# vats98754/zero-knowledge-proofs

Measured on AMD Instinct MI355X. Metric: Groth16 prove constraints/sec at 2^20 R1CS; G1 MSM throughput (scalar-point/s), higher is better.
Workload: dtype u32; 1 GPU; groth16_prove_2^20; circuit=n x (x*y=z) (groth16-cli generate_crs), field=BLS12-381 Fq/Fr Montgomery, 32x32->64-bit limb products (radix 2^28/2^29), constraints=1048576, constraints_per_gpu=1048576, num_public=1, parallelism=single-gpu, quotient=local

## Files before the change

### zero-knowledge-proofs_amd/__init__.py

```python
import ctypes as C
import os

import numpy as np

_HERE = os.path.dirname(os.path.abspath(__file__))
LIB_PATH = os.environ.get("ZK_AMD_LIB") or os.path.join(_HERE, "libzkp_amd.so")
TEST_LIB_PATH = os.path.join(os.path.dirname(LIB_PATH), "libzkp_amd_test.so")

R = 0x73EDA753299D7D483339D80809A1D80553BDA402FFFE5BFEFFFFFFFF00000001

ZK_OK, ZK_ERR_MSM_LEN, ZK_ERR_INVALID_WITNESS, ZK_ERR_QAP_DIVISION, ZK_ERR_DOMAIN, \
    ZK_ERR_SETUP_PARAMS, ZK_ERR_DEVICE, ZK_ERR_RCCL, ZK_ERR_ARG, ZK_ERR_DIMENSION = range(10)
G1_WORDS, G2_WORDS = 13, 25
PARTIAL_BYTES = 1536

EXPORTS = (
    "zk_ctx_create", "zk_ctx_destroy", "zk_last_error", "zk_ctx_synchronize",
    "zk_ctx_profile", "zk_ctx_profile_read",
    "zk_msm_g1", "zk_msm_g2", "zk_msm_g1_upload", "zk_msm_g2_upload", "zk_msm_bases_free",
    "zk_msm_g1_dev", "zk_msm_g2_dev", "zk_ntt_fr", "zk_ntt_fr_dev",
    "zk_groth16_setup", "zk_groth16_setup_dev", "zk_pk_upload", "zk_pk_free",
    "zk_groth16_prove", "zk_groth16_prove_dev", "zk_pk_upload_shard",
    "zk_groth16_setup_dev_shard", "zk_groth16_prove_partial", "zk_groth16_prove_combine",
    "zk_proof_serialize_compressed", "zk_rccl_unique_id", "zk_ctx_attach_rccl",
# ... 8 lines not shown
    "zk_groth16_verify_many", "zk_pairing_products",
    "zk_groth16_setup_sound", "zk_groth16_setup_sound_dev", "zk_pk_upload_sound", "zk_pk_is_sound",
    "zk_groth16_verify_sound", "zk_groth16_verify_many_sound",
    "zk_msm_g1_upload_copies", "zk_msm_g2_upload_copies", "zk_pk_device_bytes",
    "zk_proofs_deserialize_compressed", "zk_groth16_verify_many_bytes", "zk_groth16_verify_many_bytes_sound",
    "zk_groth16_verify_all_sound", "zk_groth16_verify_all_bytes_sound",
    "zk_g1_mul_scalar", "zk_groth16_contribute_sound", "zk_groth16_verify_contribution_sound",
    "zk_srs_generate", "zk_g1_ntt", "zk_g2_ntt", "zk_groth16_setup_srs_sound", "zk_srs_verify",
    "zk_g1_mul_scalars", "zk_g2_mul_scalars", "zk_srs_contribute", "zk_srs_verify_contribution",
    "zk_sha256", "zk_hash_to_g2_host", "zk_hash_to_g2", "zk_pok_make", "zk_pok_verify", "zk_pok_verify_many",
    "zk_srs_digest", "zk_groth16_key_digest_sound", "zk_srs_prove_contribution",
    "zk_srs_verify_contribution_proofs",
    "zk_vk_prepare", "zk_vk_dev_free", "zk_vk_dev_bytes", "zk_vk_dev_is_sound", "zk_groth16_prepare_inputs",
    "zk_groth16_verify_many_prepared", "zk_groth16_verify_many_bytes_prepared",
)
TEST_EXPORTS = ("zk_test_prove_virtual_shards", "zk_test_exchange", "zk_test_fault_after_exchange",
                "zk_test_pk_bases", "zk_test_pk_info", "zk_test_pk_plan", "zk_test_fq_sqrt", "zk_test_fq2_sqrt",
                "zk_test_fq12", "zk_test_pairing_gt", "zk_test_fixed_base_g1", "zk_test_fixed_base_g2",
                "zk_test_verify_all_parts", "zk_test_g1_mul_scalar_plain",
                "zk_test_g1_mul_scalars_plain", "zk_test_g2_mul_scalars_plain", "zk_test_g1_mul_scalars_table",
                "zk_test_g2_mul_scalars_table", "zk_test_split_scalars", "zk_test_field", "zk_test_curve",
                "zk_test_gn_walk", "zk_test_hash_to_g2_capped", "zk_test_prepared_plan", "zk_test_prepared_run",
                "zk_test_prepared_force", "zk_test_prepared_info", "zk_test_msm_force", "zk_test_msm_info",
                "zk_test_msm_grouping", "zk_test_msm_scrub")
TEST_MSM_INFO = ("c", "nwin", "bits", "sw", "shared", "copies", "nred", "nseg", "segshift", "G", "T", "fix_max",
                 "M", "nbig", "natural_T", "n")
TEST_MSM_PART_G2, TEST_MSM_PART_ABI = 5, 6
ZK_OPT_QUOTIENT_PATH, ZK_OPT_PROVE_WIN_C, ZK_OPT_EXCHANGE_TIMEOUT_MS, ZK_OPT_DIST_QUOTIENT = 1, 2, 3, 5
ZK_OPT_EXCHANGE_FIRST = 6
ZK_OPT_POINT_CHUNK = 7
ZK_OPT_VERIFY_CHUNK = 8
ZK_OPT_SOUND_WIN_C = 9
ZK_OPT_SOUND_COPIES = 10
ZK_OPT_GNTT_MAP = 12
ZK_OPT_SRS_RUN = 13
ZK_VERIFY_REJECT, ZK_VERIFY_ACCEPT, ZK_VERIFY_MALFORMED = range(3)
(ZK_TEST_FQ12_MUL, ZK_TEST_FQ12_SQR, ZK_TEST_FQ12_INV, ZK_TEST_FQ12_CONJ, ZK_TEST_FQ12_FROB1, ZK_TEST_FQ12_FROB2,
 ZK_TEST_FQ12_CYC_SQR, ZK_TEST_FQ12_LINE_MUL, ZK_TEST_FQ12_FINAL_EXP) = range(9)
FINAL_EXP_C = 3
(ZK_TEST_FIELD_FR, ZK_TEST_FIELD_FQ, ZK_TEST_FIELD_FQ2, ZK_TEST_FIELD_FQ2H, ZK_TEST_FIELD_FQC,
 ZK_TEST_FIELD_FQ2C) = range(6)
(ZK_TEST_FOP_MUL, ZK_TEST_FOP_SQR, ZK_TEST_FOP_ADD, ZK_TEST_FOP_SUB, ZK_TEST_FOP_NEG, ZK_TEST_FOP_DBL,
 ZK_TEST_FOP_INV, ZK_TEST_FOP_TO_MONT, ZK_TEST_FOP_FROM_MONT, ZK_TEST_FOP_MUL_LAZY, ZK_TEST_FOP_MUL_SUB,
 ZK_TEST_FOP_FQ_INV, ZK_TEST_FOP_IS_ZERO) = range(13)
(ZK_TEST_COP_DBL, ZK_TEST_COP_DBL_CALL, ZK_TEST_COP_AFF_DBL, ZK_TEST_COP_MADD, ZK_TEST_COP_ADD,
 ZK_TEST_COP_ADD_ILP, ZK_TEST_COP_ADD_QUAD, ZK_TEST_COP_ADD_DUO) = range(8)
TEST_FIELD_WORDS = (8, 12, 24, 24, 12, 24)
# ... 565 lines not shown
    def prepare_inputs(self, pvk, inputs):
        if isinstance(inputs, np.ndarray) and inputs.ndim == 3:
            n = len(inputs)
        else:
            inputs = list(inputs)
            n = len(inputs)
        inp = self._verify_inputs(pvk, inputs, n)
        ic = np.zeros((n, G1_WORDS), dtype=np.uint64)
        ok = np.zeros(n, dtype=np.uint8)
        rc = lib().zk_groth16_prepare_inputs(C.c_void_p(self._h), pvk._handle(), _p(inp) if inp.size else None,
                                             C.c_size_t(inp.shape[1]), C.c_size_t(n), _p(ic) if n else None,
                                             _p(ok) if n else None)
        _check(rc, self, "zk_groth16_prepare_inputs")
        return ic, ok

    def test_prepared_force(self, width=0, run=0):
        _check(test_lib().zk_test_prepared_force(C.c_void_p(self._h), C.c_int(width), C.c_uint32(run)), self,
               "zk_test_prepared_force")

    def test_msm_force(self, T=0, fix_max=0):
        _check(test_lib().zk_test_msm_force(C.c_void_p(self._h), C.c_uint32(T), C.c_uint32(fix_max)), self,
               "zk_test_msm_force")

    def test_msm_scrub(self):
        _check(test_lib().zk_test_msm_scrub(C.c_void_p(self._h)), self, "zk_test_msm_scrub")

    def test_msm_info(self, which=0, g2=False):
        v = (C.c_uint32 * len(TEST_MSM_INFO))()
        _check(test_lib().zk_test_msm_info(C.c_void_p(self._h), C.c_int(which), C.c_int(1 if g2 else 0), v), self,
               "zk_test_msm_info")
        return dict(zip(TEST_MSM_INFO, (int(x) for x in v)))

    def test_msm_grouping(self, which=0):
        G, M = C.c_size_t(), C.c_size_t()
        fn = test_lib().zk_test_msm_grouping
        _check(fn(C.c_void_p(self._h), C.c_int(which), None, None, None, C.c_size_t(0), C.byref(G), C.byref(M)),
               self, "zk_test_msm_grouping")
        cap = max(G.value + 1, M.value)
        off, key, ent = (np.zeros(cap, dtype=np.uint32) for _ in range(3))
        _check(fn(C.c_void_p(self._h), C.c_int(which), _p(off), _p(key), _p(ent), C.c_size_t(cap), C.byref(G),
                  C.byref(M)), self, "zk_test_msm_grouping")
        return off[:G.value + 1], key[:M.value], ent[:M.value]

    @staticmethod
    def _proof_bytes(data, what):
        if isinstance(data, np.ndarray):
# ... 1507 lines not shown
```

### zero-knowledge-proofs_amd/csrc/group.hip

```cpp
#include "msm.hpp"

namespace zk {

#ifndef ZK_GS_THREADS
#define ZK_GS_THREADS 512
#endif
#ifndef ZK_GS_IPT
#define ZK_GS_IPT 16
#endif
constexpr uint32_t GS_THREADS = ZK_GS_THREADS;
constexpr uint32_t GS_WAVES = GS_THREADS / 64;
constexpr uint32_t GS_IPT = ZK_GS_IPT;
constexpr uint32_t GS_TE = GS_THREADS * GS_IPT;
constexpr uint32_t GS_WR = GS_IPT;
#ifndef ZK_GS_RB
#define ZK_GS_RB 8
#endif
constexpr uint32_t GS_MAXRB = ZK_GS_RB;
constexpr uint32_t GS_MAXNB = 1u << GS_MAXRB;
constexpr uint32_t GS_SCAN_ITEMS = 8;
constexpr uint32_t GS_SCAN_THREADS = 1024;
constexpr uint32_t GS_SCAN_CHUNK = GS_SCAN_ITEMS * GS_SCAN_THREADS;

struct GsArgs {
  const uint64_t* sc[MSM_MAXSEG];
  uint32_t n[MSM_MAXSEG], wstride[MSM_MAXSEG], ioff[MSM_MAXSEG], kbase[MSM_MAXSEG];
  uint32_t tile0[MSM_MAXSEG + 1];
  uint32_t boff[MSM_MAXWIN];
  uint32_t nseg, nwin, c, bits, shared, G, M, rb;
  uint32_t copies, setstride;
};

struct GsWin {
  uint32_t copy, ebase, kbase;
};
ZK_DI GsWin gs_next_win(const GsArgs& a, GsWin gw, uint32_t ioff, uint32_t wstride) {
  const bool wrap = gw.copy + 1 == a.copies;
  return {wrap ? 0u : gw.copy + 1, wrap ? ioff : gw.ebase + wstride, wrap ? gw.kbase + a.setstride : gw.kbase};
}

template <int SW>
ZK_DI uint32_t gs_digit(const GsArgs& a, uint32_t w, const uint64_t (&s)[SW], uint32_t& carry, bool& neg) {
  const bool top = w == a.nwin - 1;
  const int width = top ? (int)(a.bits - a.c * w) : (int)a.c;
  const uint32_t v = scal_window<SW>(s, (int)(a.c * w), width) + carry;
  if (!top && v > (1u << (a.c - 1))) {
    carry = 1;
    neg = true;
    return (1u << a.c) - v;
  }
  carry = 0;
  neg = false;
  return v;
}

ZK_DI void gs_entry(const GsArgs& a, GsWin gw, uint32_t i, uint32_t w, uint32_t mag, bool neg, uint32_t& key,
                    uint32_t& ent) {
  if (a.shared) {
    key = gw.kbase + (mag ? mag - 1 : 0u);
    ent = mag ? ((gw.ebase + i) | (neg ? 0x80000000u : 0u)) : MSM_DUMMY;
  } else {
    key = mag ? a.boff[w] + mag - 1 : a.G;
    ent = i | (neg ? 0x80000000u : 0u);
  }
}

ZK_DI uint32_t gs_seg(const GsArgs& a, uint32_t tile) {
  uint32_t k = 0;
#pragma unroll
  for (uint32_t j = 1; j < MSM_MAXSEG; j++)
    if (j < a.nseg && tile >= a.tile0[j]) k = j;
  return k;
}

template <int SW, bool SRC>
ZK_DI void gs_load(const GsArgs& a, uint32_t tile, const uint32_t* __restrict__ kin, const uint32_t* __restrict__ ein,
                   uint32_t (&key)[GS_IPT], uint32_t (&ent)[GS_IPT], uint32_t& valid) {
  const uint32_t lane = threadIdx.x & 63, wave = threadIdx.x >> 6;
  valid = 0;
  if constexpr (SRC) {
    const uint32_t k = gs_seg(a, tile);
    const uint32_t u0 = (tile - a.tile0[k]) * (GS_TE / 64) + wave * GS_WR;
    const uint32_t nk = a.n[k];
    uint32_t pr = u0 / a.nwin, w = u0 - pr * a.nwin;
    uint32_t i = pr * 64 + lane;
    uint64_t s[SW];
    uint32_t carry = 0;
    bool neg = false;
#pragma unroll
    for (int j = 0; j < SW; j++) s[j] = i < nk ? a.sc[k][(size_t)i * SW + j] : 0ull;
    const uint32_t ioff = a.ioff[k], wstride = a.wstride[k];
    const GsWin gw0{0u, ioff, a.kbase[k]};
    GsWin gw = gw0;
    for (uint32_t q = 0; q < w; q++) {
      (void)gs_digit<SW>(a, q, s, carry, neg);
      gw = gs_next_win(a, gw, ioff, wstride);
    }
#pragma unroll
    for (uint32_t r = 0; r < GS_IPT; r++) {
      key[r] = ent[r] = 0;
      if (i < nk) {
        const uint32_t mag = gs_digit<SW>(a, w, s, carry, neg);
        gs_entry(a, gw, i, w, mag, neg, key[r], ent[r]);
        valid |= 1u << r;
      }
      gw = gs_next_win(a, gw, ioff, wstride);
      if (++w == a.nwin) {
        w = 0;
        carry = 0;
        gw = gw0;
        i += 64;
#pragma unroll
        for (int j = 0; j < SW; j++) s[j] = (r + 1 < GS_IPT && i < nk) ? a.sc[k][(size_t)i * SW + j] : 0ull;
      }
    }
  } else {
    const size_t e0 = (size_t)tile * GS_TE + wave * GS_WR * 64 + lane;
#pragma unroll
    for (uint32_t r = 0; r < GS_IPT; r++) {
      const size_t e = e0 + 64 * r;
      const bool ok = e < a.M;
      key[r] = ok ? kin[e] : 0u;
      ent[r] = ok ? ein[e] : 0u;
      if (ok) valid |= 1u << r;
    }
  }
}

template <int SW, bool SRC>
__global__ void __launch_bounds__(GS_THREADS) k_gs_count(GsArgs a, uint32_t shift, uint32_t ntiles,
                                                         const uint32_t* __restrict__ kin,
                                                         uint32_t* __restrict__ cnt) {
  __shared__ uint32_t h[GS_MAXNB];
  const uint32_t NB = 1u << a.rb, tile = blockIdx.x;
  for (uint32_t b = threadIdx.x; b < NB; b += GS_THREADS) h[b] = 0;
  __syncthreads();
  uint32_t key[GS_IPT], ent[GS_IPT], valid;
  if constexpr (SRC) {
    gs_load<SW, true>(a, tile, nullptr, nullptr, key, ent, valid);
  } else {
    const size_t e0 = (size_t)tile * GS_TE + (threadIdx.x >> 6) * GS_WR * 64 + (threadIdx.x & 63);
    valid = 0;
#pragma unroll
    for (uint32_t r = 0; r < GS_IPT; r++) {
// ... 143 lines not shown
    for (uint32_t bit = 0; bit < a.rb; bit++) {
      const uint64_t bb = __ballot((d >> bit) & 1u);
      m &= ((d >> bit) & 1u) ? bb : ~bb;
    }
    if (ok) {
      const uint32_t base = wh[wave][d];
      const uint32_t slot = base + __popcll(m & lt_mask);
      sk[slot] = key[r];
      se[slot] = ent[r];
      if ((m & lt_mask) == 0) wh[wave][d] = base + __popcll(m);
      cnt++;
    }
  }
  uint32_t tot = 0;
  (void)gs_block_scan<GS_THREADS>(cnt, ws, &tot);
  for (uint32_t j = threadIdx.x; j < tot; j += GS_THREADS) {
    const uint32_t k = sk[j];
    const uint32_t g = tb[(k >> shift) & (NB - 1)] + j;
    kout[g] = k;
    eout[g] = se[j];
  }
}

constexpr uint32_t OFF_LONG_RUN = 64;
__global__ void __launch_bounds__(256) k_msm_offsets(const uint32_t* __restrict__ key, uint32_t M, uint32_t G,
                                                     uint32_t* __restrict__ off, uint32_t* __restrict__ ctl) {
  __shared__ uint32_t run_lo[256], run_hi[256], run_i[256], nrun;
  const uint32_t i = blockIdx.x * blockDim.x + threadIdx.x;
  if (i < 2) ctl[i] = 0;
  if (threadIdx.x == 0) nrun = 0;
  __syncthreads();
  if (i <= M) {
    const uint32_t lo = i ? min(key[i - 1], G) + 1 : 0;
    const uint32_t hi = i < M ? min(key[i], G) : G;
    if (lo <= hi && hi - lo >= OFF_LONG_RUN) {
      const uint32_t r = atomicAdd(&nrun, 1u);
      run_lo[r] = lo;
      run_hi[r] = hi;
      run_i[r] = i;
    } else {
      for (uint32_t g = lo; g <= hi; g++) off[g] = i;
    }
  }
  __syncthreads();
  for (uint32_t r = 0; r < nrun; r++)
    for (uint32_t g = run_lo[r] + threadIdx.x; g <= run_hi[r]; g += 256) off[g] = run_i[r];
}

void msm_offsets(MsmWork& w, uint32_t M, hipStream_t st) {
  w.nbig.ensure(2 * sizeof(uint32_t));
  k_msm_offsets<<<ceil_div((uint64_t)M + 1, 256), 256, 0, st>>>(w.key.as<uint32_t>(), M, w.plan.G,
                                                                 w.off.as<uint32_t>(), w.nbig.as<uint32_t>());
  ZK_LAUNCH_CHECK();
}

template <int SW>
static void gs_run(MsmWork& w, const GsArgs& a, uint32_t ntiles0, hipStream_t st) {
  const MsmPlan& p = w.plan;
  const uint32_t M = a.M;
  uint32_t maxkey = p.shared ? p.G - 1 : p.G;
  uint32_t kb = 1;
  while (kb < 32 && (maxkey >> kb)) kb++;
  const uint32_t P = (kb + GS_MAXRB - 1) / GS_MAXRB;
  GsArgs g = a;
  g.rb = (kb + P - 1) / P;
  const uint32_t NB = 1u << g.rb;
  const uint32_t ntiles1 = ceil_div(M, GS_TE);
  const size_t L = (size_t)NB * std::max(ntiles0, ntiles1);
  w.gcnt.ensure(sizeof(uint32_t) * std::max<size_t>(L, 1));
  w.gcnt_sums.ensure(sizeof(uint32_t) * (L / GS_SCAN_CHUNK + 2));
  uint32_t* cnt = w.gcnt.as<uint32_t>();
  uint32_t* sums = w.gcnt_sums.as<uint32_t>();
  uint32_t* kbuf[2] = {w.key.as<uint32_t>(), w.key_in.as<uint32_t>()};
  uint32_t* ebuf[2] = {w.ent.as<uint32_t>(), w.ent_in.as<uint32_t>()};
  const uint32_t* kin = nullptr;
  const uint32_t* ein = nullptr;
  for (uint32_t pass = 0; pass < P; pass++) {
    const uint32_t shift = pass * g.rb;
    const uint32_t nt = pass == 0 ? ntiles0 : ntiles1;
    const size_t Lp = (size_t)NB * nt;
    if (pass == 0)
      k_gs_count<SW, true><<<nt, GS_THREADS, 0, st>>>(g, shift, nt, nullptr, cnt);
    else
      k_gs_count<SW, false><<<nt, GS_THREADS, 0, st>>>(g, shift, nt, kin, cnt);
    ZK_LAUNCH_CHECK();
    const uint32_t nchunk = ceil_div(Lp, GS_SCAN_CHUNK);
    k_gs_scan_sums<<<nchunk, GS_SCAN_THREADS, 0, st>>>(cnt, Lp, sums);
    ZK_LAUNCH_CHECK();
// ... 20 lines not shown
  a.shared = p.shared ? 1u : 0u;
  a.G = p.G;
  a.copies = p.shared ? (uint32_t)p.copies : 1u;
  a.setstride = p.nb[0];
  for (int k = 0; k < p.nwin && k < MSM_MAXWIN; k++) a.boff[k] = p.boff[k];
  uint32_t tiles = 0;
  size_t M = 0;
  for (int k = 0; k < nseg; k++) {
    a.sc[k] = segs[k].scalars;
    a.n[k] = segs[k].n;
    a.wstride[k] = segs[k].wstride ? segs[k].wstride : segs[k].n;
    a.ioff[k] = segs[k].ioff;
    a.kbase[k] = (p.shared && nseg > 1) ? (uint32_t)k << (p.segshift & 31) : 0u;
    a.tile0[k] = tiles;
    const uint64_t rounds = (uint64_t)ceil_div(segs[k].n, 64) * (uint64_t)p.nwin;
    tiles += (uint32_t)((rounds + GS_TE / 64 - 1) / (GS_TE / 64));
    M += (size_t)segs[k].n * p.nwin;
  }
  for (int k = nseg; k <= MSM_MAXSEG; k++) a.tile0[k] = tiles;
  a.M = (uint32_t)M;
  if (M) {
    w.key_in.ensure(sizeof(uint32_t) * M);
    w.ent_in.ensure(sizeof(uint32_t) * M);
    if (sw == 1) gs_run<1>(w, a, tiles, st);
    else gs_run<4>(w, a, tiles, st);
  }
  msm_offsets(w, (uint32_t)M, st);
}

}
```

### zero-knowledge-proofs_amd/csrc/msm.hip

```cpp
#include <algorithm>
#include <cstdlib>
#include <cstring>
#include <type_traits>
#include <vector>

#include "msm.hpp"

namespace zk {

MsmPlan msm_make_plan(uint32_t n, int bits, int sw, int force_c) {
  MsmPlan p{};
  p.n = n;
  p.bits = bits;
  p.sw = sw;
  int best_c = 4;
  double best = 1e300;
  for (int nw = (bits + 15) / 16; nw <= std::min(MSM_MAXWIN, bits); nw++) {
    const int c = (bits + nw - 1) / nw;
    if (c < 4) break;
    const int nwin = (bits + c - 1) / c;
    const int top = bits - c * (nwin - 1);
    const double nbuck = (double)(nwin - 1) * (1u << (c - 1)) + (double)(1u << top);
    const double cost = (double)n * nwin + 3.5 * nbuck;
    if (cost < best) { best = cost; best_c = c; }
// ... 668 lines not shown
  const uint32_t n = p.n;
  (void)n;
  int ph = pf ? pf->begin(st, (w.tag + "msm_merge").c_str(), p.G) : -1;
  const bool by_boundary = p.G > p.T;
  const size_t fix_n = by_boundary ? p.T : p.G;
  k_msm_fixup<C><<<ceil_div(Lanes<C>::N * fix_n, 128), 128, 0, st>>>(
      w.key.as<uint32_t>(), w.off.as<uint32_t>(), p.G, p.T, p.fix_max, by_boundary, w.nbig.as<uint32_t>(),
      w.buckets.as<X>(), w.partials.as<X>());
  ZK_LAUNCH_CHECK();
  {
    uint32_t nlevels = 0;
    while ((1ull << (ZK_MERGE_FAN_LOG * nlevels)) < p.T) nlevels++;
    const uint32_t groups1 = (uint32_t)(((uint64_t)p.T + MSM_MERGE_FAN - 1) >> ZK_MERGE_FAN_LOG);
    if (nlevels) {
      const uint32_t grid = std::min<uint32_t>(std::min<uint32_t>(ceil_div(groups1, 128), 64), merge_max_blocks<C>());
      if (grid < 1 || grid > merge_max_blocks<C>()) throw Error(ZK_ERR_DEVICE, "msm: merge grid exceeds residency");
      k_msm_merge<C><<<grid, 128, 0, st>>>(
          w.key.as<uint32_t>(), w.off.as<uint32_t>(), p.G, p.T, p.fix_max, nlevels, w.nbig.as<uint32_t>(),
          w.buckets.as<X>(), w.partials.as<X>(), w.partials2.as<X>());
      ZK_LAUNCH_CHECK();
    }
  }
  p.all_valid = 0;
  if (mode == MSM_BACK_COMBINE || mode == MSM_BACK_ACCUM) {
    if (!prev || prev->plan.G != p.G || prev->plan.nseg != p.nseg) throw Error(ZK_ERR_ARG, "msm: combine plans differ");
    const bool prev_all = prev->plan.all_valid != 0;
    k_msm_combine<C><<<ceil_div(Lanes<C>::N * (size_t)p.G, 128), 128, 0, st>>>(
        w.off.as<uint32_t>(), prev->off.as<uint32_t>(), prev_all, p.G, w.buckets.as<X>(), prev->buckets.as<X>());
    ZK_LAUNCH_CHECK();
    p.all_valid = 1;
  }
  if (pf) pf->end(st, ph);
  if (mode == MSM_BACK_FIXUP || mode == MSM_BACK_ACCUM) return;
  ph = pf ? pf->begin(st, (w.tag + "msm_bucket_sum").c_str(), p.G) : -1;
  k_msm_rowcol<C><<<ceil_div(p.nrc, MSM_RED_WAVES), 64 * MSM_RED_WAVES, 0, st>>>(p, w.off.as<uint32_t>(),
                                                                                w.buckets.as<X>(), w.rc.as<X>());
  ZK_LAUNCH_CHECK();
  constexpr int RW = g2 ? ZK_QUANT_WAVES_G2 : ZK_QUANT_WAVES_G1;
  k_msm_quant<C, RW><<<p.nq, 64 * RW, 0, st>>>(p, w.rc.as<X>(), w.res.as<X>());
  ZK_LAUNCH_CHECK();
  if (pf) pf->end(st, ph);
}

template <class C>
void msm_launch(MsmWork& w, const typename C::A* d_bases, const uint64_t* d_scalars, int sw, uint32_t n,
                int bits, hipStream_t st, uint32_t stride) {
  w.plan = msm_make_plan(n, bits, sw);
  const MsmSeg seg{d_bases, d_scalars, n, stride};
// ... 120 lines not shown
  out[t] = k < iw ? in[i * iw + k] : make_uint4(0, 0, 0, 0);
}

template <class C>
uint32_t msm_pad_bases(DevBuf& d, size_t n, hipStream_t st) {
  constexpr uint32_t sz = sizeof(typename C::A), padded = (sz + 127) / 128 * 128;
  if (padded == sz) return 0;
  DevBuf out;
  out.ensure((size_t)padded * std::max<size_t>(n, 1));
  if (n) {
    k_pad_copy<<<ceil_div(n * (padded / 16), 256), 256, 0, st>>>(d.as<uint4>(), n, sz / 16, padded / 16,
                                                                  out.as<uint4>());
    ZK_LAUNCH_CHECK();
  }
  ZK_HIP(hipStreamSynchronize(st));
  d = std::move(out);
  return padded;
}

template <class C>
void msm_download(MsmWork& w, hipStream_t st) {
  using X = typename C::X;
  const size_t bytes = sizeof(X) * w.plan.nq;
  w.host_res.ensure(bytes);
  ZK_HIP(hipMemcpyAsync(w.host_res.p, w.res.p, bytes, hipMemcpyDeviceToHost, st));
}

template <class C>
static host::X<typename C::HF> msm_finish_impl(const MsmWork& w, int seg) {
  using HF = typename C::HF;
  using HX = host::X<HF>;
  static_assert(sizeof(HX) == sizeof(typename C::X), "layout");
  const MsmPlan& p = w.plan;
  const HX* r = w.host_res.as<const HX>();
  auto wexp = [&](int win) { return !p.shared ? p.c * win : p.nseg > 1 ? 0 : p.c * p.copies * win; };
  const int w0 = seg < 0 ? 0 : seg, w1 = seg < 0 ? (int)p.nred : seg + 1;
  int maxe = 0;
  for (int win = w0; win < w1; win++)
    maxe = std::max(maxe, wexp(win) + std::max<int>(p.kc[win] + p.kr[win] - 1, p.kc[win]));
  std::vector<std::vector<const HX*>> at(maxe + 1);
  for (int win = w0; win < w1; win++) {
    const int kr = p.kr[win], kc = p.kc[win];
    for (int q = 0; q < kr + kc + 1; q++) {
      int e = q < kr ? wexp(win) + kc + q : q < kr + kc ? wexp(win) + (q - kr) : wexp(win);
      at[e].push_back(&r[p.qoff[win] + q]);
    }
  }
  HX acc = host::inf<HF>();
  auto host_form = [](const HX& d) {
    return HX{host::to_host(d.X_), host::to_host(d.Y), host::to_host(d.ZZ), host::to_host(d.ZZZ)};
  };
  for (int e = maxe; e >= 0; e--) {
    acc = host::dbl(acc);
    for (const HX* t : at[e]) acc = host::addp(acc, host_form(*t));
  }
  return acc;
}
// ... 104 lines not shown
```

### zero-knowledge-proofs_amd/csrc/msm.hpp

```cpp
#pragma once
#include <string>
#include <vector>

#include "common.hpp"
#include "curve.hpp"
#include "host_ec.hpp"

namespace zk {

template <int SW>
__device__ __forceinline__ uint32_t scal_window(const uint64_t (&s)[SW], int off, int width) {
  int wd = off >> 6, sh = off & 63;
  uint64_t lo = 0;
#pragma unroll
  for (int k = 0; k < SW; k++)
    if (k == wd) lo = s[k] >> sh;
  if (sh + width > 64) {
#pragma unroll
    for (int k = 0; k < SW; k++)
      if (k == wd + 1) lo |= s[k] << (64 - sh);
  }
  return (uint32_t)(lo & ((1ull << width) - 1));
}

// ... 38 lines not shown

constexpr int MSM_MAXSEG = 4;
struct MsmSeg {
  const void* bases;
  const uint64_t* scalars;
  uint32_t n;
  uint32_t stride = 0;
  uint32_t wstride = 0, ioff = 0;
};

MsmPlan msm_make_plan(uint32_t n, int bits, int sw, int force_c = 0);
struct MsmWork;
struct MsmSeg;
void msm_group(MsmWork& w, const MsmSeg* segs, int nseg, int sw, hipStream_t st);
void msm_offsets(MsmWork& w, uint32_t M, hipStream_t st);
MsmPlan msm_make_plan_shared(uint32_t n, int bits, int sw, int c);
MsmPlan msm_make_plan_grouped(uint32_t n, int bits, int sw, int c, int copies);

struct MsmWork {
  DevBuf off, ent, key, buckets, partials, partials2, rc, res;
  DevBuf key_in, ent_in;
  DevBuf nbig;
  DevBuf gcnt, gcnt_sums;
  PinnedBuf host_res;
  MsmPlan plan{};
  Prof* prof = nullptr;
  std::string tag;
  uint32_t force_T = 0, force_fix_max = 0;
};

template <class C>
uint32_t msm_accum_units();

template <class C>
void msm_launch(MsmWork& w, const typename C::A* d_bases, const uint64_t* d_scalars, int sw,
                uint32_t n, int bits, hipStream_t st, uint32_t stride = 0);
template <class C>
void msm_launch_grouped(MsmWork& w, const typename C::A* d_bases, const uint64_t* d_scalars, int sw,
                        uint32_t n, int bits, int c, int copies, hipStream_t st, uint32_t stride = 0);
template <class C>
void msm_launch_batch(MsmWork& w, const MsmSeg* segs, int nseg, int bits, int c, hipStream_t st);
enum { MSM_BACK_FULL = 0, MSM_BACK_FIXUP = 1, MSM_BACK_COMBINE = 2, MSM_BACK_ACCUM = 3 };
template <class C>
void msm_batch_front(MsmWork& w, const MsmSeg* segs, int nseg, int bits, int c, hipStream_t st);
template <class C>
void msm_batch_back(MsmWork& w, hipStream_t st, int mode, const MsmWork* prev);
template <class C>
void msm_precompute_windows(typename C::A* d_bases, size_t n, int W, int c, hipStream_t st);
template <class C>
uint32_t msm_pad_bases(DevBuf& d, size_t n, hipStream_t st);
template <class C>
void batch_normalize(const typename C::X* d_in, size_t n, typename C::F* d_pre, typename C::A* d_out,
// ... 19 lines not shown
```

### zero-knowledge-proofs_amd/csrc/testhooks.hip

```cpp
#include <algorithm>
#include <cstring>
#include <vector>

#include "ceremony.hpp"
#include "ctx.hpp"
#include "hash.hpp"
#include "msm.hpp"
#include "mulvec.hpp"
#include "pairing.hpp"
#include "points.hpp"
#include "prepared.hpp"
#include "prove.hpp"
#include "setup.hpp"
#include "verify_all.hpp"
#include "../../include/zkp_test.h"

using namespace zk;

#define ZK_TGUARD(ctx, ...)                                   \
  try {                                                       \
    ZK_HIP(hipSetDevice((ctx)->device));                      \
    __VA_ARGS__                                               \
  } catch (const zk::Error& e) {                              \
    (ctx)->err = e.what();                                    \
// ... 793 lines not shown
  return nullptr;
}
static void test_msm_sync(zk_ctx* ctx) {
  ZK_HIP(hipStreamSynchronize(ctx->stream));
  for (int k = 0; k < NUM_SIDE; k++)
    if (ctx->side[k]) ZK_HIP(hipStreamSynchronize(ctx->side[k]));
}
static bool test_msm_ran(const MsmWork& w) { return w.plan.G && w.off.p && w.nbig.p && w.key.p && w.ent.p; }
}

int zk_test_msm_force(zk_ctx* ctx, uint32_t T, uint32_t fix_max) {
  if (!ctx || T > (1u << 22)) return ZK_ERR_ARG;
  for (int k = 0; k < NUM_MSM; k++) {
    ctx->msm[k].force_T = T;
    ctx->msm[k].force_fix_max = fix_max;
  }
  for (int k = 0; k < HOST_PARTS - 1; k++) {
    ctx->part_g2[k].force_T = ctx->part_abi[k].force_T = T;
    ctx->part_g2[k].force_fix_max = ctx->part_abi[k].force_fix_max = fix_max;
  }
  return ZK_OK;
}

int zk_test_msm_info(zk_ctx* ctx, int which, int g2, uint32_t* info) {
  if (!ctx || !info || (g2 != 0 && g2 != 1)) return ZK_ERR_ARG;
  MsmWork* w = test_msm_work(ctx, which);
  if (!w) return ZK_ERR_ARG;
  ZK_TGUARD(ctx, {
    if (!test_msm_ran(*w)) throw Error(ZK_ERR_ARG, "test_msm_info: no MSM has run on this workspace");
    const MsmPlan& p = w->plan;
    test_msm_sync(ctx);
    uint32_t M = 0, nbig = 0;
    ZK_HIP(hipMemcpy(&M, w->off.as<uint32_t>() + p.G, sizeof(uint32_t), hipMemcpyDeviceToHost));
    ZK_HIP(hipMemcpy(&nbig, w->nbig.p, sizeof(uint32_t), hipMemcpyDeviceToHost));
    info[ZK_TEST_MSM_C] = (uint32_t)p.c;
    info[ZK_TEST_MSM_NWIN] = (uint32_t)p.nwin;
    info[ZK_TEST_MSM_BITS] = (uint32_t)p.bits;
    info[ZK_TEST_MSM_SW] = (uint32_t)p.sw;
    info[ZK_TEST_MSM_SHARED] = (uint32_t)p.shared;
    info[ZK_TEST_MSM_COPIES] = (uint32_t)p.copies;
    info[ZK_TEST_MSM_NRED] = p.nred;
    info[ZK_TEST_MSM_NSEG] = (uint32_t)p.nseg;
    info[ZK_TEST_MSM_SEGSHIFT] = p.segshift;
    info[ZK_TEST_MSM_G] = p.G;
    info[ZK_TEST_MSM_T] = p.T;
    info[ZK_TEST_MSM_FIX_MAX] = p.fix_max;
// ... 49 lines not shown
```

Before: 123.7 million constraints/s.

## Fuse MSM bucket radix sort with decoupled lookback and segmented key passes

Replaces the multi-kernel radix grouping of MSM bucket keys with a fused scheme. One histogram kernel computes the digit counts for every pass and the global base offsets at once. Each pass kernel then scatters using a single-pass decoupled lookback over per-tile status words, with ticket-ordered tiles. For batched shared-window MSMs it also sorts per segment on fewer key bits, which can reduce the number of passes. The cost is spin-waiting between workgroups, guarded by a poll limit and an error flag checked on the host, plus extra control memory.

```diff
diff --git a/zero-knowledge-proofs_amd/__init__.py b/zero-knowledge-proofs_amd/__init__.py
--- a/zero-knowledge-proofs_amd/__init__.py
+++ b/zero-knowledge-proofs_amd/__init__.py
@@ -54,7 +54,8 @@
                 "zk_test_g2_mul_scalars_table", "zk_test_split_scalars", "zk_test_field", "zk_test_curve",
                 "zk_test_gn_walk", "zk_test_hash_to_g2_capped", "zk_test_prepared_plan", "zk_test_prepared_run",
                 "zk_test_prepared_force", "zk_test_prepared_info", "zk_test_msm_force", "zk_test_msm_info",
-                "zk_test_msm_grouping", "zk_test_msm_scrub")
+                "zk_test_msm_grouping", "zk_test_msm_scrub", "zk_test_group_force",
+                "zk_test_msm_batch_front", "zk_test_group_info")
 TEST_MSM_INFO = ("c", "nwin", "bits", "sw", "shared", "copies", "nred", "nseg", "segshift", "G", "T", "fix_max",
                  "M", "nbig", "natural_T", "n")
 TEST_MSM_PART_G2, TEST_MSM_PART_ABI = 5, 6
@@ -666,6 +667,23 @@
         _check(test_lib().zk_test_msm_force(C.c_void_p(self._h), C.c_uint32(T), C.c_uint32(fix_max)), self,
                "zk_test_msm_force")
 
+    def test_group_force(self, mode=0):
+        _check(test_lib().zk_test_group_force(C.c_void_p(self._h), C.c_int(mode)), self, "zk_test_group_force")
+
+    def test_group_info(self, which=0):
+        f, e = C.c_uint32(), C.c_uint32()
+        _check(test_lib().zk_test_group_info(C.c_void_p(self._h), C.c_int(which), C.byref(f), C.byref(e)), self,
+               "zk_test_group_info")
+        return bool(f.value), int(e.value)
+
+    def test_msm_batch_front(self, scalars, sizes):
+        sc = np.ascontiguousarray(scalars, dtype=np.uint64).reshape(-1)
+        n = np.asarray(sizes, dtype=np.uint32)
+        if int(n.sum()) != len(sc):
+            raise ValueError("test_msm_batch_front: sizes do not add up to the scalars")
+        _check(test_lib().zk_test_msm_batch_front(C.c_void_p(self._h), _p(sc) if len(sc) else None, _p(n),
+                                                  C.c_int(len(n))), self, "zk_test_msm_batch_front")
+
     def test_msm_scrub(self):
         _check(test_lib().zk_test_msm_scrub(C.c_void_p(self._h)), self, "zk_test_msm_scrub")
 
diff --git a/zero-knowledge-proofs_amd/csrc/group.hip b/zero-knowledge-proofs_amd/csrc/group.hip
--- a/zero-knowledge-proofs_amd/csrc/group.hip
+++ b/zero-knowledge-proofs_amd/csrc/group.hip
@@ -18,6 +18,9 @@
 #endif
 constexpr uint32_t GS_MAXRB = ZK_GS_RB;
 constexpr uint32_t GS_MAXNB = 1u << GS_MAXRB;
+#ifndef ZK_GS_SEGMENTED
+#define ZK_GS_SEGMENTED 1
+#endif
 constexpr uint32_t GS_SCAN_ITEMS = 8;
 constexpr uint32_t GS_SCAN_THREADS = 1024;
 constexpr uint32_t GS_SCAN_CHUNK = GS_SCAN_ITEMS * GS_SCAN_THREADS;
@@ -26,6 +29,7 @@
   const uint64_t* sc[MSM_MAXSEG];
   uint32_t n[MSM_MAXSEG], wstride[MSM_MAXSEG], ioff[MSM_MAXSEG], kbase[MSM_MAXSEG];
   uint32_t tile0[MSM_MAXSEG + 1];
+  uint32_t tile1[MSM_MAXSEG + 1], soff[MSM_MAXSEG + 1], nts;
   uint32_t boff[MSM_MAXWIN];
   uint32_t nseg, nwin, c, bits, shared, G, M, rb;
   uint32_t copies, setstride;
@@ -70,6 +74,13 @@
 #pragma unroll
   for (uint32_t j = 1; j < MSM_MAXSEG; j++)
     if (j < a.nseg && tile >= a.tile0[j]) k = j;
+  return k;
+}
+ZK_DI uint32_t gs_seg1(const GsArgs& a, uint32_t tile) {
+  uint32_t k = 0;
+#pragma unroll
+  for (uint32_t j = 1; j < MSM_MAXSEG; j++)
+    if (j < a.nts && tile >= a.tile1[j]) k = j;
   return k;
 }
 
@@ -115,11 +126,13 @@
       }
     }
   } else {
-    const size_t e0 = (size_t)tile * GS_TE + wave * GS_WR * 64 + lane;
+    const uint32_t k = gs_seg1(a, tile);
+    const size_t e0 = a.soff[k] + (size_t)(tile - a.tile1[k]) * GS_TE + wave * GS_WR * 64 + lane;
+    const size_t end = a.soff[k + 1];
 #pragma unroll
     for (uint32_t r = 0; r < GS_IPT; r++) {
       const size_t e = e0 + 64 * r;
-      const bool ok = e < a.M;
+      const bool ok = e < end;
       key[r] = ok ? kin[e] : 0u;
       ent[r] = ok ? ein[e] : 0u;
       if (ok) valid |= 1u << r;
@@ -309,11 +322,225 @@
   }
 }
 
+constexpr uint32_t GS_MAXP = 4;
+constexpr uint32_t GS_CTL_ERR = 0, GS_CTL_ARRIVED = 1, GS_CTL_TICKET = 2, GS_CTL_HIST = 8;
+constexpr uint32_t GS_HIST_WORDS = GS_MAXP * MSM_MAXSEG * GS_MAXNB;
+constexpr uint32_t GS_CTL_BASE = GS_CTL_HIST + GS_HIST_WORDS;
+constexpr uint32_t GS_CTL_STAT = GS_CTL_BASE + GS_HIST_WORDS;
+constexpr bool GS_FUSED_OK = GS_MAXNB <= GS_THREADS && GS_MAXRB * GS_MAXP >= 32;
+
+constexpr uint32_t GS_ST_SHIFT = 30, GS_ST_MASK = (1u << GS_ST_SHIFT) - 1;
+constexpr uint32_t GS_ST_AGG = 1, GS_ST_INCL = 2, GS_ST_BLOCK = 3;
+constexpr uint32_t GS_LB = 16;
+constexpr uint32_t GS_BLK = 32;
+constexpr uint32_t GS_POLL_MAX = 1u << 20;
+
+#ifndef ZK_GS_RELEASE
+#define ZK_GS_RELEASE 0
+#endif
+ZK_DI void gs_publish(uint32_t* p, uint32_t state, uint32_t count) {
+  __hip_atomic_store(p, state << GS_ST_SHIFT | count, ZK_GS_RELEASE ? __ATOMIC_RELEASE : __ATOMIC_RELAXED,
+                     __HIP_MEMORY_SCOPE_AGENT);
+}
+
+template <uint32_t STEP>
+ZK_DI bool gs_walk(uint32_t* stat, uint32_t NB, uint32_t b, uint32_t pos, uint32_t n, uint32_t& sum, bool& incl) {
+  uint32_t polls = 0;
+  while (n && !incl) {
+    uint32_t wv[GS_LB];
+#pragma unroll
+    for (uint32_t j = 0; j < GS_LB; j++)
+      wv[j] = j < n ? __hip_atomic_load(&stat[(size_t)(pos - STEP * j) * NB + b], __ATOMIC_RELAXED,
+                                        __HIP_MEMORY_SCOPE_AGENT)
+                    : 0u;
+    bool stall = false;
+    uint32_t adv = 0;
+#pragma unroll
+    for (uint32_t j = 0; j < GS_LB; j++) {
+      const uint32_t st = wv[j] >> GS_ST_SHIFT;
+      if (j < n && !incl && !stall) {
+        if (STEP == 1 ? st == 0 : st < GS_ST_INCL) {
+          stall = true;
+        } else {
+          sum += wv[j] & GS_ST_MASK;
+          adv++;
+          incl = st == GS_ST_INCL;
+        }
+      }
+    }
+    n -= adv;
+    pos -= STEP * adv;
+    if (stall) {
+      if (++polls > GS_POLL_MAX) return false;
+      __builtin_amdgcn_s_sleep(4);
+    }
+  }
+  return true;
+}
+
+ZK_DI bool gs_lookback(uint32_t* stat, uint32_t NB, uint32_t b, uint32_t first, uint32_t tile, uint32_t tc,
+                       uint32_t& excl) {
+  const uint32_t rel = tile - first, blk = rel / GS_BLK, in_blk = rel % GS_BLK;
+  uint32_t sum = 0;
+  bool incl = false;
+  if (!gs_walk<1>(stat, NB, b, tile - 1, in_blk, sum, incl)) return false;
+  if (!incl && blk) {
+    if (in_blk == GS_BLK - 1) gs_publish(&stat[(size_t)tile * NB + b], GS_ST_BLOCK, sum + tc);
+    if (!gs_walk<GS_BLK>(stat, NB, b, tile - in_blk - 1, blk, sum, incl)) return false;
+  }
+  if (ZK_GS_RELEASE) __builtin_amdgcn_fence(__ATOMIC_ACQUIRE, "agent");
+  excl = sum;
+  return true;
+}
+
+template <int SW>
+__global__ void __launch_bounds__(GS_THREADS) k_gs_hist(GsArgs a, uint32_t P, uint32_t nrows,
+                                                        uint32_t* __restrict__ ctl) {
+  __shared__ uint32_t h[GS_MAXP][GS_MAXNB];
+  __shared__ uint32_t ws[GS_THREADS / 64 + 1];
+  __shared__ uint32_t last;
+  const uint32_t NB = 1u << a.rb, tile = blockIdx.x;
+  for (uint32_t j = threadIdx.x; j < GS_MAXP * GS_MAXNB; j += GS_THREADS) (&h[0][0])[j] = 0;
+  __syncthreads();
+  uint32_t key[GS_IPT], ent[GS_IPT], valid;
+  gs_load<SW, true>(a, tile, nullptr, nullptr, key, ent, valid);
+  (void)ent;
+#pragma unroll
+  for (uint32_t r = 0; r < GS_IPT; r++)
+    if (valid >> r & 1u)
+      for (uint32_t p = 0; p < P; p++) atomicAdd(&h[p][(key[r] >> (p * a.rb)) & (NB - 1)], 1u);
+  __syncthreads();
+  uint32_t* hist = ctl + GS_CTL_HIST;
+  const uint32_t reg = a.nts > 1 ? gs_seg(a, tile) : 0u;
+  for (uint32_t j = threadIdx.x; j < P * NB; j += GS_THREADS) {
+    const uint32_t p = j >> a.rb, b = j & (NB - 1), c = h[p][b];
+    if (c) __hip_atomic_fetch_add(&hist[(p * MSM_MAXSEG + reg) * GS_MAXNB + b], c, __ATOMIC_RELAXED,
+                                  __HIP_MEMORY_SCOPE_AGENT);
+  }
+  uint32_t* stat = ctl + GS_CTL_STAT;
+  const size_t nstat = (size_t)2 * nrows * NB;
+  for (size_t j = (size_t)blockIdx.x * GS_THREADS + threadIdx.x; j < nstat; j += (size_t)gridDim.x * GS_THREADS)
+    stat[j] = 0;
+  __threadfence();
+  __syncthreads();
+  if (threadIdx.x == 0)
+    last = __hip_atomic_fetch_add(&ctl[GS_CTL_ARRIVED], 1u, __ATOMIC_ACQ_REL, __HIP_MEMORY_SCOPE_AGENT) ==
+           gridDim.x - 1;
+  __syncthreads();
+  if (!last) return;
+  __threadfence();
+  uint32_t* base = ctl + GS_CTL_BASE;
+  for (uint32_t p = 0; p < P; p++)
+    for (uint32_t k = 0; k < a.nts; k++) {
+      uint32_t* hp = &hist[(p * MSM_MAXSEG + k) * GS_MAXNB];
+      uint32_t c = 0;
+      if (threadIdx.x < NB) {
+        c = __hip_atomic_load(&hp[threadIdx.x], __ATOMIC_RELAXED, __HIP_MEMORY_SCOPE_AGENT);
+        __hip_atomic_store(&hp[threadIdx.x], 0u, __ATOMIC_RELAXED, __HIP_MEMORY_SCOPE_AGENT);
+      }
+      const uint32_t ex = gs_block_scan<GS_THREADS>(c, ws, nullptr);
+      if (threadIdx.x < NB) base[(p * MSM_MAXSEG + k) * GS_MAXNB + threadIdx.x] = a.soff[k] + ex;
+    }
+  if (threadIdx.x < GS_MAXP) ctl[GS_CTL_TICKET + threadIdx.x] = 0;
+  if (threadIdx.x == 0) ctl[GS_CTL_ERR] = ctl[GS_CTL_ARRIVED] = 0;
+}
+
+template <int SW, bool SRC>
+__global__ void __launch_bounds__(GS_THREADS) k_gs_pass(GsArgs a, uint32_t pass, uint32_t* __restrict__ ctl,
+                                                        uint32_t* __restrict__ stat, uint32_t* __restrict__ clr,
+                                                        const uint32_t* __restrict__ kin,
+                                                        const uint32_t* __restrict__ ein,
+                                                        uint32_t* __restrict__ kout, uint32_t* __restrict__ eout) {
+  static_assert(GS_MAXNB <= GS_THREADS || !GS_FUSED_OK, "a thread per bin");
+  __shared__ uint32_t sk[GS_TE], se[GS_TE];
+  __shared__ uint32_t wh[GS_WAVES][GS_MAXNB];
+  __shared__ uint32_t tb[GS_MAXNB];
+  __shared__ uint32_t ws[GS_THREADS / 64 + 1];
+  __shared__ uint32_t my_tile, gave_up;
+  const uint32_t NB = 1u << a.rb, shift = pass * a.rb;
+  const uint32_t lane = threadIdx.x & 63, wave = threadIdx.x >> 6;
+  if (threadIdx.x == 0) {
+    my_tile = __hip_atomic_fetch_add(&ctl[GS_CTL_TICKET + pass], 1u, __ATOMIC_RELAXED, __HIP_MEMORY_SCOPE_AGENT);
+    gave_up = 0;
+  }
+  for (uint32_t j = threadIdx.x; j < GS_WAVES * GS_MAXNB; j += GS_THREADS) (&wh[0][0])[j] = 0;
+  __syncthreads();
+  const uint32_t tile = my_tile;
+  uint32_t reg = 0, first = 0;
+  if (a.nts > 1) {
+    reg = SRC ? gs_seg(a, tile) : gs_seg1(a, tile);
+    first = SRC ? a.tile0[reg] : a.tile1[reg];
+  }
+  uint32_t key[GS_IPT], ent[GS_IPT], valid;
+  gs_load<SW, SRC>(a, tile, kin, ein, key, ent, valid);
+#pragma unroll
+  for (uint32_t r = 0; r < GS_IPT; r++)
+    if (valid >> r & 1u) atomicAdd(&wh[wave][(key[r] >> shift) & (NB - 1)], 1u);
+  __syncthreads();
+  const uint32_t b = threadIdx.x;
+  uint32_t tc = 0;
+  if (b < NB) {
+    for (uint32_t v = 0; v < GS_WAVES; v++) {
+      const uint32_t c = wh[v][b];
+      wh[v][b] = tc;
+      tc += c;
+    }
+    gs_publish(&stat[(size_t)tile * NB + b], tile == first ? GS_ST_INCL : GS_ST_AGG, tc);
+    if (clr) clr[(size_t)tile * NB + b] = 0;
+  }
+  const uint32_t lb = gs_block_scan<GS_THREADS>(tc, ws, nullptr);
+  if (b < NB) {
+    uint32_t excl = 0;
+    if (tile != first) {
+      if (gs_lookback(stat, NB, b, first, tile, tc, excl)) {
+        gs_publish(&stat[(size_t)tile * NB + b], GS_ST_INCL, excl + tc);
+      } else {
+        __hip_atomic_store(&ctl[GS_CTL_ERR], 1u, __ATOMIC_RELAXED, __HIP_MEMORY_SCOPE_AGENT);
+        gave_up = 1;
+      }
+    }
+    tb[b] = ctl[GS_CTL_BASE + (pass * MSM_MAXSEG + reg) * GS_MAXNB + b] + excl - lb;
+    for (uint32_t v = 0; v < GS_WAVES; v++) wh[v][b] += lb;
+  }
+  __syncthreads();
+  if (gave_up) return;
+  const uint64_t lt_mask = (1ull << lane) - 1;
+  uint32_t cnt = 0;
+#pragma unroll
+  for (uint32_t r = 0; r < GS_IPT; r++) {
+    const bool ok = valid >> r & 1u;
+    const uint32_t d = (key[r] >> shift) & (NB - 1);
+    uint64_t m = __ballot(ok);
+    for (uint32_t bit = 0; bit < a.rb; bit++) {
+      const uint64_t bb = __ballot((d >> bit) & 1u);
+      m &= ((d >> bit) & 1u) ? bb : ~bb;
+    }
+    if (ok) {
+      const uint32_t base = wh[wave][d];
+      const uint32_t slot = base + __popcll(m & lt_mask);
+      sk[slot] = key[r];
+      se[slot] = ent[r];
+      if ((m & lt_mask) == 0) wh[wave][d] = base + __popcll(m);
+      cnt++;
+    }
+  }
+  uint32_t tot = 0;
+  (void)gs_block_scan<GS_THREADS>(cnt, ws, &tot);
+  for (uint32_t j = threadIdx.x; j < tot; j += GS_THREADS) {
+    const uint32_t k = sk[j];
+    const uint32_t g = tb[(k >> shift) & (NB - 1)] + j;
+    kout[g] = k;
+    eout[g] = se[j];
+  }
+}
+
 constexpr uint32_t OFF_LONG_RUN = 64;
 __global__ void __launch_bounds__(256) k_msm_offsets(const uint32_t* __restrict__ key, uint32_t M, uint32_t G,
-                                                     uint32_t* __restrict__ off, uint32_t* __restrict__ ctl) {
+                                                     uint32_t* __restrict__ off, uint32_t* __restrict__ ctl,
+                                                     const uint32_t* __restrict__ err) {
   __shared__ uint32_t run_lo[256], run_hi[256], run_i[256], nrun;
   const uint32_t i = blockIdx.x * blockDim.x + threadIdx.x;
+  if (err && *err) M = 0;
   if (i < 2) ctl[i] = 0;
   if (threadIdx.x == 0) nrun = 0;
   __syncthreads();
@@ -336,9 +563,67 @@
 
 void msm_offsets(MsmWork& w, uint32_t M, hipStream_t st) {
   w.nbig.ensure(2 * sizeof(uint32_t));
+  const uint32_t* err = w.group_fused ? w.gctl.as<uint32_t>() + GS_CTL_ERR : nullptr;
   k_msm_offsets<<<ceil_div((uint64_t)M + 1, 256), 256, 0, st>>>(w.key.as<uint32_t>(), M, w.plan.G,
-                                                                 w.off.as<uint32_t>(), w.nbig.as<uint32_t>());
+                                                                 w.off.as<uint32_t>(), w.nbig.as<uint32_t>(), err);
   ZK_LAUNCH_CHECK();
+}
+
+template <int SW>
+static void gs_run_fused(MsmWork& w, const GsArgs& a, uint32_t ntiles0, hipStream_t st) {
+  const MsmPlan& p = w.plan;
+  GsArgs g = a;
+  const bool batch = a.nseg > 1 && a.shared && ZK_GS_SEGMENTED;
+  uint32_t kb = 1;
+  if (batch) {
+    kb = p.segshift;
+  } else {
+    const uint32_t maxkey = p.shared ? p.G - 1 : p.G;
+    while (kb < 32 && (maxkey >> kb)) kb++;
+  }
+  const uint32_t P = (kb + GS_MAXRB - 1) / GS_MAXRB;
+  g.rb = (kb + P - 1) / P;
+  const uint32_t NB = 1u << g.rb;
+  g.nts = batch ? a.nseg : 1u;
+  uint32_t ntiles1 = 0, at = 0;
+  for (uint32_t k = 0; k < g.nts; k++) {
+    const uint32_t len = batch ? a.n[k] * a.nwin : a.M;
+    g.soff[k] = at;
+    g.tile1[k] = ntiles1;
+    at += len;
+    ntiles1 += ceil_div(len, GS_TE);
+  }
+  for (uint32_t k = g.nts; k <= MSM_MAXSEG; k++) {
+    g.soff[k] = at;
+    g.tile1[k] = ntiles1;
+  }
+  const uint32_t nrows = std::max(ntiles0, ntiles1);
+  const size_t words = GS_CTL_STAT + (size_t)2 * nrows * NB;
+  if (w.gctl.bytes < sizeof(uint32_t) * words) {
+    w.gctl.ensure(sizeof(uint32_t) * words);
+    ZK_HIP(hipMemsetAsync(w.gctl.p, 0, sizeof(uint32_t) * GS_CTL_BASE, st));
+  }
+  uint32_t* ctl = w.gctl.as<uint32_t>();
+  uint32_t* stat[2] = {ctl + GS_CTL_STAT, ctl + GS_CTL_STAT + (size_t)nrows * NB};
+  k_gs_hist<SW><<<ntiles0, GS_THREADS, 0, st>>>(g, P, nrows, ctl);
+  ZK_LAUNCH_CHECK();
+  uint32_t* kbuf[2] = {w.key.as<uint32_t>(), w.key_in.as<uint32_t>()};
+  uint32_t* ebuf[2] = {w.ent.as<uint32_t>(), w.ent_in.as<uint32_t>()};
+  const uint32_t* kin = nullptr;
+  const uint32_t* ein = nullptr;
+  for (uint32_t pass = 0; pass < P; pass++) {
+    const uint32_t out = (P - 1 - pass) & 1u;
+    uint32_t* clr = pass >= 1 && pass + 1 < P ? stat[(pass + 1) & 1u] : nullptr;
+    if (pass == 0)
+      k_gs_pass<SW, true><<<ntiles0, GS_THREADS, 0, st>>>(g, pass, ctl, stat[0], clr, nullptr, nullptr, kbuf[out],
+                                                          ebuf[out]);
+    else
+      k_gs_pass<SW, false><<<ntiles1, GS_THREADS, 0, st>>>(g, pass, ctl, stat[pass & 1u], clr, kin, ein, kbuf[out],
+                                                           ebuf[out]);
+    ZK_LAUNCH_CHECK();
+    kin = kbuf[out];
+    ein = ebuf[out];
+  }
 }
 
 template <int SW>
@@ -351,6 +636,9 @@
   const uint32_t P = (kb + GS_MAXRB - 1) / GS_MAXRB;
   GsArgs g = a;
   g.rb = (kb + P - 1) / P;
+  g.nts = 1;
+  g.tile1[0] = g.soff[0] = 0;
+  for (uint32_t k = 1; k <= MSM_MAXSEG; k++) g.soff[k] = M;
   const uint32_t NB = 1u << g.rb;
   const uint32_t ntiles1 = ceil_div(M, GS_TE);
   const size_t L = (size_t)NB * std::max(ntiles0, ntiles1);
@@ -417,8 +705,16 @@
   if (M) {
     w.key_in.ensure(sizeof(uint32_t) * M);
     w.ent_in.ensure(sizeof(uint32_t) * M);
-    if (sw == 1) gs_run<1>(w, a, tiles, st);
-    else gs_run<4>(w, a, tiles, st);
+    w.group_fused = GS_FUSED_OK && M < (1ull << GS_ST_SHIFT) && w.force_group != 1;
+    if (w.group_fused) {
+      if (sw == 1) gs_run_fused<1>(w, a, tiles, st);
+      else gs_run_fused<4>(w, a, tiles, st);
+    } else {
+      if (sw == 1) gs_run<1>(w, a, tiles, st);
+      else gs_run<4>(w, a, tiles, st);
+    }
+  } else {
+    w.group_fused = false;
   }
   msm_offsets(w, (uint32_t)M, st);
 }
diff --git a/zero-knowledge-proofs_amd/csrc/msm.hip b/zero-knowledge-proofs_amd/csrc/msm.hip
--- a/zero-knowledge-proofs_amd/csrc/msm.hip
+++ b/zero-knowledge-proofs_amd/csrc/msm.hip
@@ -714,8 +714,10 @@
     }
   }
   p.all_valid = 0;
+  w.err_prev = nullptr;
   if (mode == MSM_BACK_COMBINE || mode == MSM_BACK_ACCUM) {
     if (!prev || prev->plan.G != p.G || prev->plan.nseg != p.nseg) throw Error(ZK_ERR_ARG, "msm: combine plans differ");
+    w.err_prev = prev;
     const bool prev_all = prev->plan.all_valid != 0;
     k_msm_combine<C><<<ceil_div(Lanes<C>::N * (size_t)p.G, 128), 128, 0, st>>>(
         w.off.as<uint32_t>(), prev->off.as<uint32_t>(), prev_all, p.G, w.buckets.as<X>(), prev->buckets.as<X>());
@@ -882,8 +884,17 @@
 void msm_download(MsmWork& w, hipStream_t st) {
   using X = typename C::X;
   const size_t bytes = sizeof(X) * w.plan.nq;
-  w.host_res.ensure(bytes);
+  w.host_res.ensure(bytes + sizeof(uint32_t) * MSM_MAX_ERR_WORDS);
   ZK_HIP(hipMemcpyAsync(w.host_res.p, w.res.p, bytes, hipMemcpyDeviceToHost, st));
+  w.err_at = bytes;
+  w.err_n = 0;
+  for (const MsmWork* q = &w; q; q = q->err_prev) {
+    if (!q->group_fused) continue;
+    if (w.err_n == MSM_MAX_ERR_WORDS) throw Error(ZK_ERR_ARG, "msm: too many parts");
+    ZK_HIP(hipMemcpyAsync(static_cast<char*>(w.host_res.p) + bytes + sizeof(uint32_t) * w.err_n, q->gctl.p,
+                          sizeof(uint32_t), hipMemcpyDeviceToHost, st));
+    w.err_n++;
+  }
 }
 
 template <class C>
@@ -893,6 +904,9 @@
   static_assert(sizeof(HX) == sizeof(typename C::X), "layout");
   const MsmPlan& p = w.plan;
   const HX* r = w.host_res.as<const HX>();
+  const uint32_t* err = reinterpret_cast<const uint32_t*>(static_cast<const char*>(w.host_res.p) + w.err_at);
+  for (uint32_t k = 0; k < w.err_n; k++)
+    if (err[k]) throw Error(ZK_ERR_DEVICE, "msm: the bucket grouping timed out waiting for an earlier tile");
   auto wexp = [&](int win) { return !p.shared ? p.c * win : p.nseg > 1 ? 0 : p.c * p.copies * win; };
   const int w0 = seg < 0 ? 0 : seg, w1 = seg < 0 ? (int)p.nred : seg + 1;
   int maxe = 0;
diff --git a/zero-knowledge-proofs_amd/csrc/msm.hpp b/zero-knowledge-proofs_amd/csrc/msm.hpp
--- a/zero-knowledge-proofs_amd/csrc/msm.hpp
+++ b/zero-knowledge-proofs_amd/csrc/msm.hpp
@@ -84,12 +84,19 @@
   DevBuf key_in, ent_in;
   DevBuf nbig;
   DevBuf gcnt, gcnt_sums;
+  DevBuf gctl;
+  bool group_fused = false;
+  const MsmWork* err_prev = nullptr;
+  size_t err_at = 0;
+  uint32_t err_n = 0;
   PinnedBuf host_res;
   MsmPlan plan{};
   Prof* prof = nullptr;
   std::string tag;
   uint32_t force_T = 0, force_fix_max = 0;
+  int force_group = 0;
 };
+constexpr uint32_t MSM_MAX_ERR_WORDS = 8;
 
 template <class C>
 uint32_t msm_accum_units();
diff --git a/zero-knowledge-proofs_amd/csrc/testhooks.hip b/zero-knowledge-proofs_amd/csrc/testhooks.hip
--- a/zero-knowledge-proofs_amd/csrc/testhooks.hip
+++ b/zero-knowledge-proofs_amd/csrc/testhooks.hip
@@ -839,6 +839,55 @@
   return ZK_OK;
 }
 
+int zk_test_group_force(zk_ctx* ctx, int mode) {
+  if (!ctx || mode < 0 || mode > 2) return ZK_ERR_ARG;
+  for (int k = 0; k < NUM_MSM; k++) ctx->msm[k].force_group = mode;
+  for (int k = 0; k < HOST_PARTS - 1; k++) ctx->part_g2[k].force_group = ctx->part_abi[k].force_group = mode;
+  return ZK_OK;
+}
+
+int zk_test_group_info(zk_ctx* ctx, int which, uint32_t* fused, uint32_t* gave_up) {
+  if (!ctx || !fused || !gave_up) return ZK_ERR_ARG;
+  MsmWork* w = test_msm_work(ctx, which);
+  if (!w) return ZK_ERR_ARG;
+  ZK_TGUARD(ctx, {
+    if (!test_msm_ran(*w)) throw Error(ZK_ERR_ARG, "test_group_info: no MSM has run on this workspace");
+    test_msm_sync(ctx);
+    *fused = w->group_fused ? 1u : 0u;
+    *gave_up = 0;
+    if (w->group_fused) ZK_HIP(hipMemcpy(gave_up, w->gctl.p, sizeof(uint32_t), hipMemcpyDeviceToHost));
+    return ZK_OK;
+  })
+}
+
+int zk_test_msm_batch_front(zk_ctx* ctx, const uint64_t* scalars, const uint32_t* n, int nseg) {
+  if (!ctx || !n || nseg < 1 || nseg > MSM_MAXSEG) return ZK_ERR_ARG;
+  size_t total = 0;
+  for (int k = 0; k < nseg; k++) total += n[k];
+  if ((total && !scalars) || total > (1u << 24)) return ZK_ERR_ARG;
+  ZK_TGUARD(ctx, {
+    constexpr int C = 16, NWIN = 4;
+    test_msm_sync(ctx);
+    DevBuf bases, sc;
+    bases.ensure(sizeof(G1A) * NWIN * std::max<size_t>(total, 1));
+    sc.ensure(sizeof(uint64_t) * std::max<size_t>(total, 1));
+    ZK_HIP(hipMemsetAsync(bases.p, 0, bases.bytes, ctx->stream));
+    if (total)
+      ZK_HIP(hipMemcpyAsync(sc.p, scalars, sizeof(uint64_t) * total, hipMemcpyHostToDevice, ctx->stream));
+    MsmSeg segs[MSM_MAXSEG];
+    uint32_t at = 0;
+    for (int k = 0; k < nseg; k++) {
+      segs[k] = MsmSeg{bases.p, sc.as<uint64_t>() + at, n[k]};
+      segs[k].wstride = (uint32_t)total;
+      segs[k].ioff = at;
+      at += n[k];
+    }
+    msm_batch_front<G1>(ctx->msm[0], segs, nseg, 64, C, ctx->stream);
+    ZK_HIP(hipStreamSynchronize(ctx->stream));
+    return ZK_OK;
+  })
+}
+
 int zk_test_msm_info(zk_ctx* ctx, int which, int g2, uint32_t* info) {
   if (!ctx || !info || (g2 != 0 && g2 != 1)) return ZK_ERR_ARG;
   MsmWork* w = test_msm_work(ctx, which);
```

New measurement: 110.1 million constraints/s. 11.0% lower.
